# nv-legate/legate.sparse

Measured on AMD Instinct MI355X. Metric: cg_iters_per_sec, higher is better.
Workload: dtype fp64; 1 GPU; model=poisson2d-5pt-cg, nx=16384, n=268435456, nnz=1342111744, parallelism=dp1 1-D row partition + window gather

## Files before the change

### sparse/kernels/src/common.h

```cpp
#pragma once

#include <type_traits>

#include <hip/hip_runtime.h>

#include <ATen/ATen.h>
#include <ATen/Dispatch.h>
#include <ATen/hip/HIPContext.h>
#include <c10/util/complex.h>

#define SPARSE_CHECK_HIP(cmd)                                             \
  do {                                                                    \
    hipError_t e = (cmd);                                                 \
    TORCH_CHECK(e == hipSuccess, "HIP error: ", hipGetErrorString(e));    \
  } while (0)

constexpr int WAVE = 64;

__device__ __forceinline__ int64_t ub_i64(const int64_t* arr, int64_t n, int64_t key) {
  int64_t lo = 0, hi = n;
  while (lo < hi) {
    int64_t mid = (lo + hi) >> 1;
    if (arr[mid] <= key) lo = mid + 1; else hi = mid;
  }
  return lo;
}

__device__ __forceinline__ int64_t lb_i64(const int64_t* arr, int64_t n, int64_t key) {
  int64_t lo = 0, hi = n;
  while (lo < hi) {
    int64_t mid = (lo + hi) >> 1;
    if (arr[mid] < key) lo = mid + 1; else hi = mid;
  }
  return lo;
}

template <typename T>
__device__ __forceinline__ void atomic_add_any(T* addr, T v) {
  atomicAdd(addr, v);
}
template <typename T>
__device__ __forceinline__ void atomic_add_any(c10::complex<T>* addr, c10::complex<T> v) {
  T* p = reinterpret_cast<T*>(addr);
  atomicAdd(p, v.real());
  atomicAdd(p + 1, v.imag());
}

template <typename T>
struct ZeroOf { static __device__ __forceinline__ T value() { return T(0); } };
template <typename T>
struct ZeroOf<c10::complex<T>> {
  static __device__ __forceinline__ c10::complex<T> value() { return {T(0), T(0)}; }
};

#define DISPATCH_INDEX(ITYPE, NAME, ...)                       \
  [&] {                                                        \
    if ((ITYPE) == at::kInt) {                                 \
      using index_t = int32_t;                                 \
      return __VA_ARGS__();                                    \
    } else {                                                   \
      using index_t = int64_t;                                 \
      return __VA_ARGS__();                                    \
    }                                                          \
  }()

#define DISPATCH_VALUES(VTYPE, NAME, ...) \
  AT_DISPATCH_FLOATING_AND_COMPLEX_TYPES(VTYPE, NAME, __VA_ARGS__)

__device__ __forceinline__ int64_t xcd_swizzle(int64_t bid, int64_t nwg) {
  constexpr int64_t NXCD = 8;
  int64_t q = nwg / NXCD, rr = nwg % NXCD;
  int64_t xcd = bid % NXCD, idx = bid / NXCD;
  return (xcd < rr ? xcd * (q + 1) : rr * (q + 1) + (xcd - rr) * q) + idx;
}

inline hipStream_t cur_stream() {
  return c10::hip::getCurrentHIPStreamMasqueradingAsCUDA().stream();
}

template <typename T>
__device__ __forceinline__ T nt_load(const T* __restrict__ p) {
  if constexpr (std::is_arithmetic_v<T>) {
    return __builtin_nontemporal_load(p);
  } else {
    return *p;
  }
}
```

### sparse/kernels/src/elemwise.hip

```cpp
#include "common.h"

namespace {

template <typename index_t>
__global__ void add_nnz_kernel(const int64_t* __restrict__ aip,
                               const index_t* __restrict__ aix,
                               const int64_t* __restrict__ bip,
                               const index_t* __restrict__ bix,
                               int64_t* __restrict__ out, int64_t m) {
  int64_t r = (int64_t)blockIdx.x * blockDim.x + threadIdx.x;
  if (r >= m) return;
  int64_t pa = aip[r], ea = aip[r + 1];
  int64_t pb = bip[r], eb = bip[r + 1];
  int64_t c = 0;
  while (pa < ea && pb < eb) {
    index_t ca = aix[pa], cb = bix[pb];
    if (ca == cb) { ++pa; ++pb; }
    else if (ca < cb) ++pa;
    else ++pb;
    ++c;
  }
  out[r] = c + (ea - pa) + (eb - pb);
}

// ... 144 lines not shown
                         dim3(256), 0, cur_stream(), aip.data_ptr<int64_t>(),
                         aix.data_ptr<index_t>(), av.data_ptr<T>(),
                         bip.data_ptr<int64_t>(), bix.data_ptr<index_t>(),
                         bv.data_ptr<T>(), cip.data_ptr<int64_t>(),
                         cix.data_ptr<index_t>(), cv.data_ptr<T>(), m,
                         static_cast<T>(alpha), static_cast<T>(beta));
    });
  });
}

void mult_nnz_hip(at::Tensor aip, at::Tensor aix, at::Tensor bip, at::Tensor bix,
                  at::Tensor out) {
  int64_t m = out.numel();
  if (m == 0) return;
  DISPATCH_INDEX(aix.scalar_type(), "mult_nnz", [&] {
    hipLaunchKernelGGL((mult_nnz_kernel<index_t>), dim3((m + 255) / 256), dim3(256),
                       0, cur_stream(), aip.data_ptr<int64_t>(),
                       aix.data_ptr<index_t>(), bip.data_ptr<int64_t>(),
                       bix.data_ptr<index_t>(), out.data_ptr<int64_t>(), m);
  });
}

void mult_compute_hip(at::Tensor aip, at::Tensor aix, at::Tensor av,
                      at::Tensor bip, at::Tensor bix, at::Tensor bv,
                      at::Tensor cip, at::Tensor cix, at::Tensor cv) {
  int64_t m = aip.numel() - 1;
  if (m == 0) return;
  DISPATCH_VALUES(cv.scalar_type(), "mult_compute", [&] {
    using T = scalar_t;
    DISPATCH_INDEX(aix.scalar_type(), "mult_compute_idx", [&] {
      hipLaunchKernelGGL((mult_compute_kernel<T, index_t>), dim3((m + 255) / 256),
                         dim3(256), 0, cur_stream(), aip.data_ptr<int64_t>(),
                         aix.data_ptr<index_t>(), av.data_ptr<T>(),
                         bip.data_ptr<int64_t>(), bix.data_ptr<index_t>(),
                         bv.data_ptr<T>(), cip.data_ptr<int64_t>(),
                         cix.data_ptr<index_t>(), cv.data_ptr<T>(), m);
    });
  });
}

void mult_dense_hip(at::Tensor indptr, at::Tensor indices, at::Tensor vals,
                    at::Tensor D, at::Tensor out) {
  int64_t nnz = vals.numel();
  if (nnz == 0) return;
  int64_t m = indptr.numel() - 1;
  DISPATCH_VALUES(vals.scalar_type(), "mult_dense", [&] {
    using T = scalar_t;
    DISPATCH_INDEX(indices.scalar_type(), "mult_dense_idx", [&] {
      hipLaunchKernelGGL((mult_dense_kernel<T, index_t>), dim3((nnz + 255) / 256),
                         dim3(256), 0, cur_stream(), indptr.data_ptr<int64_t>(),
                         indices.data_ptr<index_t>(), vals.data_ptr<T>(),
                         D.data_ptr<T>(), out.data_ptr<T>(), m, D.size(1), nnz);
    });
  });
}

void axpby_hip(at::Tensor y, at::Tensor x, at::Tensor a, at::Tensor b,
               bool isalpha, bool negate) {
  int64_t n = y.numel();
  if (n == 0) return;
  const int64_t ept = std::max<int64_t>(1, 16 / y.element_size());
  int64_t blocks = (n / ept + 255) / 256 + 1;
  DISPATCH_VALUES(y.scalar_type(), "axpby", [&] {
    using T = scalar_t;
    auto launch = [&](auto kern) {
      hipLaunchKernelGGL(kern, dim3(blocks), dim3(256), 0, cur_stream(),
                         y.data_ptr<T>(), x.data_ptr<T>(), a.data_ptr<T>(),
                         b.data_ptr<T>(), n);
    };
    if (isalpha && !negate) launch(axpby_kernel<T, true, false>);
    else if (isalpha && negate) launch(axpby_kernel<T, true, true>);
    else if (!isalpha && !negate) launch(axpby_kernel<T, false, false>);
    else launch(axpby_kernel<T, false, true>);
  });
}

namespace {

template <typename T, bool ISALPHA, bool NEG>
__global__ __launch_bounds__(256) void axpby_norm2_kernel(
    T* __restrict__ y, const T* __restrict__ x, const T* __restrict__ a,
    const T* __restrict__ b, T* __restrict__ dot_partial, int64_t n) {
  constexpr int EPT = EptOf<T>::value;
  __shared__ T red[256];
  T s = (*a) / (*b);
  if (NEG) s = -s;
  T acc = T(0);
  const int64_t nv = n / EPT;
  const int64_t i = (int64_t)blockIdx.x * blockDim.x + threadIdx.x;
  if (i < nv) {
    auto* y2 = reinterpret_cast<VVec<T>*>(y);
    auto* x2 = reinterpret_cast<const VVec<T>*>(x);
    VVec<T> yv = y2[i];
    const VVec<T> xv = x2[i];
#pragma unroll
    for (int j = 0; j < EPT; ++j) {
      yv.v[j] = ISALPHA ? (yv.v[j] + s * xv.v[j]) : (xv.v[j] + s * yv.v[j]);
      acc += yv.v[j] * yv.v[j];
    }
    y2[i] = yv;
  }
  if (blockIdx.x == 0 && threadIdx.x == 0) {
    for (int64_t t = nv * EPT; t < n; ++t) {
      T v = ISALPHA ? (y[t] + s * x[t]) : (x[t] + s * y[t]);
      y[t] = v;
      acc += v * v;
    }
  }
  red[threadIdx.x] = acc;
  __syncthreads();
  for (int w = 128; w > 0; w >>= 1) {
    if (threadIdx.x < w) red[threadIdx.x] += red[threadIdx.x + w];
    __syncthreads();
  }
  if (threadIdx.x == 0) dot_partial[blockIdx.x] = red[0];
}

template <typename T>
__global__ __launch_bounds__(256) void cg_xr_norm2_kernel(
    T* __restrict__ x, const T* __restrict__ p, T* __restrict__ r,
    const T* __restrict__ q, const T* __restrict__ a, const T* __restrict__ b,
    T* __restrict__ dot_partial, int64_t n) {
  constexpr int EPT = EptOf<T>::value;
  __shared__ T red[256];
  const T s = (*a) / (*b);
  T acc = T(0);
  const int64_t nv = n / EPT;
  const int64_t i = (int64_t)blockIdx.x * blockDim.x + threadIdx.x;
  if (i < nv) {
    auto* x2 = reinterpret_cast<VVec<T>*>(x);
    auto* r2 = reinterpret_cast<VVec<T>*>(r);
    auto* p2 = reinterpret_cast<const VVec<T>*>(p);
    auto* q2 = reinterpret_cast<const VVec<T>*>(q);
    VVec<T> xv = x2[i];
    VVec<T> rv = r2[i];
    const VVec<T> pv = p2[i];
    const VVec<T> qv = q2[i];
#pragma unroll
    for (int j = 0; j < EPT; ++j) {
      xv.v[j] += s * pv.v[j];
      rv.v[j] -= s * qv.v[j];
      acc += rv.v[j] * rv.v[j];
    }
    x2[i] = xv;
    r2[i] = rv;
  }
  if (blockIdx.x == 0 && threadIdx.x == 0) {
    for (int64_t t = nv * EPT; t < n; ++t) {
      x[t] += s * p[t];
      const T rv = r[t] - s * q[t];
      r[t] = rv;
      acc += rv * rv;
    }
  }
  red[threadIdx.x] = acc;
  __syncthreads();
  for (int w = 128; w > 0; w >>= 1) {
    if ((int)threadIdx.x < w) red[threadIdx.x] += red[threadIdx.x + w];
    __syncthreads();
  }
  if (threadIdx.x == 0) dot_partial[blockIdx.x] = red[0];
}

}

void cg_xr_norm2_hip(at::Tensor x, at::Tensor p, at::Tensor r, at::Tensor q,
                     at::Tensor a, at::Tensor b, at::Tensor dot_out) {
  int64_t n = x.numel();
  if (n == 0) return;
  const int64_t ept = std::max<int64_t>(1, 16 / x.element_size());
  int64_t blocks = (n / ept + 255) / 256 + 1;
  TORCH_CHECK(dot_out.numel() >= blocks,
              "cg_xr_norm2: dot_out too small (", dot_out.numel(), " < ",
              blocks, ")");
  AT_DISPATCH_FLOATING_TYPES(x.scalar_type(), "cg_xr_norm2", [&] {
    using T = scalar_t;
    hipLaunchKernelGGL(cg_xr_norm2_kernel<T>, dim3(blocks), dim3(256), 0,
                       cur_stream(), x.data_ptr<T>(), p.data_ptr<T>(),
                       r.data_ptr<T>(), q.data_ptr<T>(), a.data_ptr<T>(),
                       b.data_ptr<T>(), dot_out.data_ptr<T>(), n);
  });
}

void axpby_norm2_hip(at::Tensor y, at::Tensor x, at::Tensor a, at::Tensor b,
                     bool isalpha, bool negate, at::Tensor dot_out) {
  int64_t n = y.numel();
  if (n == 0) return;
  const int64_t ept = std::max<int64_t>(1, 16 / y.element_size());
  int64_t blocks = (n / ept + 255) / 256 + 1;
  TORCH_CHECK(dot_out.numel() >= blocks,
              "axpby_norm2: dot_out too small (", dot_out.numel(), " < ",
              blocks, ")");
  AT_DISPATCH_FLOATING_TYPES(y.scalar_type(), "axpby_norm2", [&] {
    using T = scalar_t;
    auto launch = [&](auto kern) {
      hipLaunchKernelGGL(kern, dim3(blocks), dim3(256), 0, cur_stream(),
                         y.data_ptr<T>(), x.data_ptr<T>(), a.data_ptr<T>(),
                         b.data_ptr<T>(), dot_out.data_ptr<T>(), n);
    };
    if (isalpha && !negate) launch(axpby_norm2_kernel<T, true, false>);
    else if (isalpha && negate) launch(axpby_norm2_kernel<T, true, true>);
    else if (!isalpha && !negate) launch(axpby_norm2_kernel<T, false, false>);
    else launch(axpby_norm2_kernel<T, false, true>);
  });
}
```

### sparse/kernels/src/spmv.hip

```cpp
#include <type_traits>

#include "common.h"

namespace {

constexpr int BLK = 256;
constexpr int VT = 8;
constexpr int64_t NNZ_PER_BLOCK = (int64_t)BLK * VT;

template <typename U>
struct alignas(4 * sizeof(U) <= 16 ? 4 * sizeof(U) : 16) Quad {
  U v[4];
};

template <typename U>
struct alignas(2 * sizeof(U) <= 16 ? 2 * sizeof(U) : 16) Pair {
  U a, b;
};

template <typename T>
__device__ __forceinline__ void block_reduce_sum(T* red, int tid) {
  __syncthreads();
  for (int w = BLK / 2; w > 0; w >>= 1) {
    if (tid < w) red[tid] += red[tid + w];
// ... 341 lines not shown
          x0 = t.a;
          x1 = t.b;
        } else {
          x0 = own[c0];
          x1 = own[c0 + 1];
        }
      } else {
        x0 = own[min(max(c0, (int64_t)0), wsize - 1)];
        x1 = own[min(max(c0 + 1, (int64_t)0), wsize - 1)];
      }
    } else {
      x0 = at<false>(min(max(c0, (int64_t)0), wsize - 1));
      x1 = at<false>(min(max(c0 + 1, (int64_t)0), wsize - 1));
    }
  }
};

template <typename T, typename index_t, bool SINGLE>
__device__ __forceinline__ void ell_accumulate(
    const index_t* __restrict__ eidx, const T* __restrict__ evals, int W,
    int64_t mp, int64_t r0, int64_t col_lo, const XWindow<T>& win, T& a0,
    T& a1) {
  for (int k = 0; k < W; ++k) {
    const int64_t base = (int64_t)k * mp + r0;
    Pair<index_t> ii;
    ii.a = nt_load(&eidx[base]);
    ii.b = nt_load(&eidx[base + 1]);
    Pair<T> vv;
    vv.a = nt_load(&evals[base]);
    vv.b = nt_load(&evals[base + 1]);
    a0 += vv.a * win.template at<SINGLE>((int64_t)ii.a - col_lo);
    a1 += vv.b * win.template at<SINGLE>((int64_t)ii.b - col_lo);
  }
}

template <typename T>
struct DiaPlanes {
  static constexpr int kBatch = 1;
  const T* __restrict__ dvals;
  int64_t mp;

  struct Rows {
    const T* __restrict__ p;
    int64_t mp;
    __device__ __forceinline__ void at(int k, T& v0, T& v1) const {
      const int64_t base = (int64_t)k * mp;
      v0 = nt_load(&p[base]);
      v1 = nt_load(&p[base + 1]);
    }
  };
  __device__ __forceinline__ Rows rows(int64_t r0) const {
    return {dvals + r0, mp};
  }
};

template <int BYTES> struct UIntOf;
template <> struct UIntOf<2> { using type = uint16_t; };
template <> struct UIntOf<4> { using type = uint32_t; };
template <> struct UIntOf<8> { using type = uint64_t; };

template <typename T, typename M>
struct DiaConstPlanes {
  static constexpr int kBatch = 8;
  const T* __restrict__ cvals;
  const M* __restrict__ mask;

  struct Rows {
    const T* __restrict__ c;
    uint32_t m0, m1;
    __device__ __forceinline__ void at(int k, T& v0, T& v1) const {
      const T ck = c[k];
      const uint32_t bit = 1u << k;
      v0 = (m0 & bit) ? ck : T(0);
      v1 = (m1 & bit) ? ck : T(0);
    }
  };
  __device__ __forceinline__ Rows rows(int64_t r0) const {
    using M2 = typename UIntOf<2 * sizeof(M)>::type;
    const M2 w = nt_load(reinterpret_cast<const M2*>(&mask[r0]));
    return {cvals, (uint32_t)(M)w, (uint32_t)(w >> (8 * sizeof(M)))};
  }
};

template <typename T, typename Planes, typename XPair>
__device__ __forceinline__ void dia_accumulate(
    const Planes& planes, const int64_t* __restrict__ offs, int W, int64_t r0,
    int64_t cbase, XPair xpair, T& a0, T& a1) {
  const auto rows = planes.rows(r0);
  constexpr int U = Planes::kBatch;
  if constexpr (U == 1) {
    for (int k = 0; k < W; ++k) {
      T v0, v1;
      rows.at(k, v0, v1);
      T x0, x1;
      xpair(cbase + offs[k], x0, x1);
      a0 += v0 * x0;
      a1 += v1 * x1;
    }
  } else {
    for (int k = 0; k < W; k += U) {
      T x0[U], x1[U];
#pragma unroll
      for (int j = 0; j < U; ++j) {
        if (k + j < W) xpair(cbase + offs[k + j], x0[j], x1[j]);
      }
#pragma unroll
      for (int j = 0; j < U; ++j) {
        if (k + j < W) {
          T v0, v1;
          rows.at(k + j, v0, v1);
          a0 += v0 * x0[j];
          a1 += v1 * x1[j];
        }
      }
    }
  }
}

template <typename T>
__device__ __forceinline__ void store_pair_or_tail(T* __restrict__ dst,
                                                   int64_t r0, int64_t m,
                                                   int64_t rhi, T v0, T v1) {
  if (r0 + 1 < min(m, rhi)) {
    *reinterpret_cast<Pair<T>*>(&dst[r0]) = Pair<T>{v0, v1};
  } else if (r0 < m) {
    dst[r0] = v0;
  }
}

template <typename T>
__device__ __forceinline__ void jacobi_update(
    const T* __restrict__ xloc, const T* __restrict__ b,
    const T* __restrict__ dinv, T* __restrict__ xout, T omega, int64_t r0,
    int64_t m, int64_t rhi, T a0, T a1) {
  if (r0 + 1 < min(m, rhi)) {
    const Pair<T> xv = *reinterpret_cast<const Pair<T>*>(&xloc[r0]);
    const Pair<T> bv = *reinterpret_cast<const Pair<T>*>(&b[r0]);
    const Pair<T> dv = *reinterpret_cast<const Pair<T>*>(&dinv[r0]);
    *reinterpret_cast<Pair<T>*>(&xout[r0]) =
        Pair<T>{xv.a + omega * dv.a * (bv.a - a0),
                xv.b + omega * dv.b * (bv.b - a1)};
  } else if (r0 < m) {
    xout[r0] = xloc[r0] + omega * dinv[r0] * (b[r0] - a0);
  }
}

template <typename T>
__device__ __forceinline__ void block_dot_partial(T* red, T d,
                                                  T* __restrict__ dot_partial) {
  red[threadIdx.x] = d;
  block_reduce_sum(red, (int)threadIdx.x);
  if (threadIdx.x == 0) dot_partial[blockIdx.x] = red[0];
}

template <typename T, typename index_t, bool FUSE_DOT, bool SINGLE>
__global__ __launch_bounds__(BLK) void ell_spmv_kernel(
    const index_t* __restrict__ eidx, const T* __restrict__ evals,
    const XWindow<T> win, T* __restrict__ y, const T* __restrict__ pvec,
    T* __restrict__ dot_partial, int64_t m, int64_t mp, int W, int64_t col_lo,
    int64_t rbase, int64_t rhi) {
  __shared__ __align__(16) char red_raw[BLK * sizeof(T)];
  const int64_t r0 = rbase + 2 * ((int64_t)blockIdx.x * BLK + threadIdx.x);
  T a0 = ZeroOf<T>::value(), a1 = ZeroOf<T>::value();
  if (r0 < rhi) {
    ell_accumulate<T, index_t, SINGLE>(eidx, evals, W, mp, r0, col_lo, win,
                                       a0, a1);
    store_pair_or_tail(y, r0, m, rhi, a0, a1);
  }
  if (FUSE_DOT) {
    T d = ZeroOf<T>::value();
    if (r0 < min(m, rhi)) d += a0 * pvec[r0];
    if (r0 + 1 < min(m, rhi)) d += a1 * pvec[r0 + 1];
    block_dot_partial(reinterpret_cast<T*>(red_raw), d, dot_partial);
  }
}

template <typename T, typename index_t, bool SINGLE>
__global__ __launch_bounds__(BLK) void ell_jacobi_kernel(
    const index_t* __restrict__ eidx, const T* __restrict__ evals,
    const XWindow<T> win, const T* __restrict__ xloc,
    const T* __restrict__ b, const T* __restrict__ dinv,
    T* __restrict__ xout, int64_t m, int64_t mp, int W, int64_t col_lo,
    T omega) {
  const int64_t r0 = 2 * ((int64_t)blockIdx.x * BLK + threadIdx.x);
  if (r0 >= mp) return;
  T a0 = ZeroOf<T>::value(), a1 = ZeroOf<T>::value();
  ell_accumulate<T, index_t, SINGLE>(eidx, evals, W, mp, r0, col_lo, win, a0,
                                     a1);
  jacobi_update(xloc, b, dinv, xout, omega, r0, m, m, a0, a1);
}

template <typename T, typename Planes, bool FUSE_DOT, bool SINGLE,
          bool RESID = false>
__global__ __launch_bounds__(BLK) void dia_spmv_kernel(
    const Planes planes,
    const int64_t* __restrict__ offs,
    const XWindow<T> win, T* __restrict__ y, const T* __restrict__ pvec,
    T* __restrict__ dot_partial, int64_t m, int64_t mp, int W, int64_t col_lo,
    int64_t row0, int64_t rbase, int64_t rhi) {
  __shared__ __align__(16) char red_raw[BLK * sizeof(T)];
  const int64_t r0 = rbase + 2 * ((int64_t)blockIdx.x * BLK + threadIdx.x);
  T a0 = ZeroOf<T>::value(), a1 = ZeroOf<T>::value();
  if (r0 < rhi) {
    dia_accumulate(
        planes, offs, W, r0, row0 + r0 - col_lo,
        [&](int64_t c0, T& x0, T& x1) {
          win.template pair<SINGLE, Planes::kBatch != 1>(c0, x0, x1);
        },
        a0, a1);
    if (!RESID) {
      store_pair_or_tail(y, r0, m, rhi, a0, a1);
    } else if (r0 + 1 < min(m, rhi)) {
      const Pair<T> bv = *reinterpret_cast<const Pair<T>*>(&pvec[r0]);
      *reinterpret_cast<Pair<T>*>(&y[r0]) = Pair<T>{bv.a - a0, bv.b - a1};
    } else if (r0 < m) {
      y[r0] = pvec[r0] - a0;
    }
  }
  if (FUSE_DOT) {
    T d = ZeroOf<T>::value();
    if (r0 < min(m, rhi)) d += a0 * pvec[r0];
    if (r0 + 1 < min(m, rhi)) d += a1 * pvec[r0 + 1];
    block_dot_partial(reinterpret_cast<T*>(red_raw), d, dot_partial);
  }
}

template <typename T, typename Planes, bool SINGLE>
__global__ __launch_bounds__(BLK) void dia_jacobi_kernel(
    const Planes planes, const int64_t* __restrict__ offs,
    const XWindow<T> win, const T* __restrict__ xloc,
    const T* __restrict__ b, const T* __restrict__ dinv,
    T* __restrict__ xout, int64_t m, int64_t mp, int W, int64_t col_lo,
    int64_t row0, T omega, int64_t rbase, int64_t rhi) {
  const int64_t r0 = rbase + 2 * ((int64_t)blockIdx.x * BLK + threadIdx.x);
  if (r0 >= rhi) return;
  T a0 = ZeroOf<T>::value(), a1 = ZeroOf<T>::value();
  dia_accumulate(
      planes, offs, W, r0, row0 + r0 - col_lo,
      [&](int64_t c0, T& x0, T& x1) {
        win.template pair<SINGLE, Planes::kBatch != 1>(c0, x0, x1);
      },
      a0, a1);
  jacobi_update(xloc, b, dinv, xout, omega, r0, m, rhi, a0, a1);
}

template <typename T, typename Planes, bool SINGLE>
__global__ __launch_bounds__(BLK) void dia_spmv_bpdot_kernel(
    const Planes planes, const int64_t* __restrict__ offs,
    const XWindow<T> rwin, const XWindow<T> pwin, T* __restrict__ pnew,
    T* __restrict__ q, const T* __restrict__ beta_num,
    const T* __restrict__ beta_den, T* __restrict__ dot_partial, int64_t m,
    int64_t mp, int W, int64_t col_lo, int64_t row0) {
  __shared__ __align__(16) char red_raw[BLK * sizeof(T)];
  const T beta = (*beta_num) / (*beta_den);
  const int64_t r0 = 2 * ((int64_t)blockIdx.x * BLK + threadIdx.x);
  T a0 = ZeroOf<T>::value(), a1 = ZeroOf<T>::value();
  T p0 = ZeroOf<T>::value(), p1 = ZeroOf<T>::value();
  if (r0 < mp) {
    auto pnew_pair = [&](int64_t c0, T& x0, T& x1) {
      T r0v, r1v, p0v, p1v;
      rwin.template pair<SINGLE, Planes::kBatch != 1>(c0, r0v, r1v);
      pwin.template pair<SINGLE, Planes::kBatch != 1>(c0, p0v, p1v);
      x0 = r0v + beta * p0v;
      x1 = r1v + beta * p1v;
    };
    const int64_t cbase = row0 + r0 - col_lo;
    dia_accumulate(planes, offs, W, r0, cbase, pnew_pair, a0, a1);
    pnew_pair(cbase, p0, p1);
    store_pair_or_tail(pnew, r0, m, m, p0, p1);
    store_pair_or_tail(q, r0, m, m, a0, a1);
  }
  T d = ZeroOf<T>::value();
  if (r0 < m) d += a0 * p0;
  if (r0 + 1 < m) d += a1 * p1;
  block_dot_partial(reinterpret_cast<T*>(red_raw), d, dot_partial);
}

inline int64_t pair_blocks(int64_t span) {
  return (span + 2 * BLK - 1) / (2 * BLK);
}

template <typename F>
void dispatch_bool(bool v, F&& f) {
  if (v) f(std::true_type{}); else f(std::false_type{});
}

struct RowPairLaunch {
  int64_t mp, rbase, rhi, nlo, nown, wsize, nblocks;
  bool single;

  RowPairLaunch(int64_t mp_, const at::Tensor& hlo, const at::Tensor& own,
                const at::Tensor& hhi, int64_t wsize_, int64_t rbase_ = 0,
                int64_t rhi_ = -1)
      : mp(mp_), rbase(rbase_), rhi(rhi_ < 0 ? mp : rhi_),
        nlo(hlo.numel()), nown(own.numel()), wsize(wsize_),
        nblocks(rhi > rbase ? pair_blocks(rhi - rbase) : 0),
        single(nlo == 0 && hhi.numel() == 0) {}

  bool empty() const { return nblocks == 0; }

  template <typename T>
  XWindow<T> window(const at::Tensor& hlo, const at::Tensor& own,
                    const at::Tensor& hhi) const {
    const T* o = own.data_ptr<T>();
    return {hlo.numel() ? hlo.data_ptr<T>() : o, o,
            hhi.numel() ? hhi.data_ptr<T>() : o, nlo, nown, wsize};
  }

  template <typename... P, typename... A>
  void launch(void (*kern)(P...), A... args) const {
    hipLaunchKernelGGL(kern, dim3(nblocks), dim3(BLK), 0, cur_stream(),
                       static_cast<P>(args)...);
  }
};

using OptTensor = c10::optional<at::Tensor>;

inline int64_t dia_mp(const at::Tensor& planes, const OptTensor& mask,
                      int64_t W) {
  return mask ? mask->numel() : planes.numel() / W;
}

template <typename T, typename F>
void dispatch_dia_planes(const at::Tensor& planes, const OptTensor& mask,
                         int64_t W, F&& f) {
  if (!mask) {
    f(DiaPlanes<T>{planes.data_ptr<T>(), planes.numel() / W});
    return;
  }
  if constexpr (std::is_floating_point_v<T>) {
    TORCH_CHECK(planes.numel() == W && W <= 8 * (int64_t)mask->element_size() &&
                    mask->numel() % 2 == 0,
                "dia: W constants and an even number of mask words of at "
                "least W bits expected");
    const T* c = planes.data_ptr<T>();
    const void* mw = mask->data_ptr();
    switch (mask->scalar_type()) {
      case at::kByte:
        f(DiaConstPlanes<T, uint8_t>{c, static_cast<const uint8_t*>(mw)});
        return;
      case at::kUInt16:
        f(DiaConstPlanes<T, uint16_t>{c, static_cast<const uint16_t*>(mw)});
        return;
      case at::kUInt32:
        f(DiaConstPlanes<T, uint32_t>{c, static_cast<const uint32_t*>(mw)});
        return;
      default:
        break;
    }
  }
  TORCH_CHECK(false, "dia: constant planes need a real value type and a "
                     "uint8/uint16/uint32 row mask");
}

}

void build_ell_hip(at::Tensor indptr, at::Tensor indices, at::Tensor values,
                   at::Tensor eidx, at::Tensor evals, int64_t W,
                   int64_t pad_idx) {
  const int64_t m = indptr.numel() - 1;
  const int64_t mp = evals.numel() / W;
  DISPATCH_VALUES(values.scalar_type(), "build_ell", [&] {
    using T = scalar_t;
    DISPATCH_INDEX(indices.scalar_type(), "build_ell_idx", [&] {
      hipLaunchKernelGGL((build_ell_kernel<T, index_t>), dim3((mp + 255) / 256),
                         dim3(256), 0, cur_stream(), indptr.data_ptr<int64_t>(),
                         indices.data_ptr<index_t>(), values.data_ptr<T>(),
                         eidx.data_ptr<index_t>(), evals.data_ptr<T>(), m, mp,
                         (int)W, (index_t)pad_idx);
    });
  });
}

void build_dia_hip(at::Tensor indptr, at::Tensor indices, at::Tensor values,
                   at::Tensor offs, at::Tensor dvals, int64_t W,
                   int64_t row0) {
  const int64_t m = indptr.numel() - 1;
  const int64_t mp = dvals.numel() / W;
  if (m == 0) return;
  DISPATCH_VALUES(values.scalar_type(), "build_dia", [&] {
    using T = scalar_t;
    DISPATCH_INDEX(indices.scalar_type(), "build_dia_idx", [&] {
      hipLaunchKernelGGL((build_dia_kernel<T, index_t>),
                         dim3((m + 255) / 256), dim3(256), 0, cur_stream(),
                         indptr.data_ptr<int64_t>(),
                         indices.data_ptr<index_t>(), values.data_ptr<T>(),
                         offs.data_ptr<int64_t>(), dvals.data_ptr<T>(), m, mp,
                         (int)W, row0);
    });
  });
}

void dia_classify_hip(at::Tensor dvals, at::Tensor cvals, at::Tensor mask,
                      at::Tensor ok, int64_t W) {
  const int64_t mp = mask.numel();
  TORCH_CHECK(dvals.numel() == W * mp && cvals.numel() == W &&
                  cvals.scalar_type() == dvals.scalar_type() &&
                  ok.scalar_type() == at::kInt &&
                  W <= 8 * (int64_t)mask.element_size(),
              "dia_classify: inconsistent arguments");
  if (mp == 0) return;
  const dim3 g1((unsigned)std::min<int64_t>((mp + 255) / 256, 1024),
                (unsigned)W);
  auto run = [&](auto bits, auto word) {
    using B = decltype(bits);
    using M = decltype(word);
    const B* d = static_cast<const B*>(dvals.data_ptr());
    B* c = static_cast<B*>(cvals.data_ptr());
    hipLaunchKernelGGL((dia_plane_const_kernel<B>), g1, dim3(256), 0,
                       cur_stream(), d, c, mp);
    hipLaunchKernelGGL((dia_row_mask_kernel<B, M>), dim3((mp + 255) / 256),
                       dim3(256), 0, cur_stream(), d, c,
                       static_cast<M*>(mask.data_ptr()),
                       ok.data_ptr<int32_t>(), mp, (int)W);
  };
  auto by_word = [&](auto bits) {
    switch (mask.scalar_type()) {
      case at::kByte: run(bits, uint8_t{}); break;
      case at::kUInt16: run(bits, uint16_t{}); break;
      case at::kUInt32: run(bits, uint32_t{}); break;
      default: TORCH_CHECK(false, "dia_classify: mask must be uint8/16/32");
    }
  };
  switch (dvals.scalar_type()) {
    case at::kFloat: by_word(uint32_t{}); break;
    case at::kDouble: by_word(uint64_t{}); break;
    default: TORCH_CHECK(false, "dia_classify: fp32/fp64 planes only");
  }
}

static at::Tensor sum_or_zero(const at::Tensor& partial,
                              const at::Tensor& like) {
  return partial.defined() ? partial.sum() : at::zeros({}, like.options());
}

// ... 1 lines not shown
                                const at::Tensor& hlo, const at::Tensor& own,
                                const at::Tensor& hhi, at::Tensor& y,
                                const at::Tensor* pvec, int64_t W, int64_t m,
                                int64_t col_lo, int64_t rbase, int64_t rhi) {
  const RowPairLaunch L(evals.numel() / W, hlo, own, hhi, 0, rbase, rhi);
  at::Tensor partial;
  if (L.empty()) return partial;
  if (pvec) partial = at::empty({L.nblocks}, evals.options());
  DISPATCH_VALUES(evals.scalar_type(), "ell_spmv", [&] {
    using T = scalar_t;
    DISPATCH_INDEX(eidx.scalar_type(), "ell_spmv_idx", [&] {
      dispatch_bool(pvec != nullptr, [&](auto fuse) {
        dispatch_bool(L.single, [&](auto single) {
          L.launch(ell_spmv_kernel<T, index_t, decltype(fuse)::value,
                                   decltype(single)::value>,
                   eidx.data_ptr<index_t>(), evals.data_ptr<T>(),
                   L.window<T>(hlo, own, hhi), y.data_ptr<T>(),
                   pvec ? pvec->data_ptr<T>() : nullptr,
                   pvec ? partial.data_ptr<T>() : nullptr, m, L.mp, W, col_lo,
                   L.rbase, L.rhi);
        });
      });
    });
  });
  return partial;
}

void ell_spmv_plain_hip(at::Tensor eidx, at::Tensor evals, at::Tensor hlo,
                        at::Tensor own, at::Tensor hhi, at::Tensor y,
                        int64_t W, int64_t m, int64_t col_lo,
                        int64_t rbase, int64_t rhi) {
  ell_spmv_impl(eidx, evals, hlo, own, hhi, y, nullptr, W, m, col_lo, rbase,
                rhi);
}

at::Tensor ell_spmv_dot_hip(at::Tensor eidx, at::Tensor evals, at::Tensor hlo,
                            at::Tensor own, at::Tensor hhi, at::Tensor y,
                            at::Tensor pvec, int64_t W, int64_t m,
                            int64_t col_lo, int64_t rbase, int64_t rhi) {
  return sum_or_zero(ell_spmv_impl(eidx, evals, hlo, own, hhi, y, &pvec, W, m,
                                   col_lo, rbase, rhi),
                     evals);
}

void ell_jacobi_hip(at::Tensor eidx, at::Tensor evals, at::Tensor hlo,
                    at::Tensor own, at::Tensor hhi, at::Tensor xloc,
                    at::Tensor b, at::Tensor dinv, at::Tensor xout,
                    int64_t W, int64_t m, int64_t col_lo, double omega) {
  const RowPairLaunch L(evals.numel() / W, hlo, own, hhi, 0);
  if (L.empty()) return;
  DISPATCH_VALUES(evals.scalar_type(), "ell_jacobi", [&] {
    using T = scalar_t;
    DISPATCH_INDEX(eidx.scalar_type(), "ell_jacobi_idx", [&] {
      dispatch_bool(L.single, [&](auto single) {
        L.launch(ell_jacobi_kernel<T, index_t, decltype(single)::value>,
                 eidx.data_ptr<index_t>(), evals.data_ptr<T>(),
                 L.window<T>(hlo, own, hhi), xloc.data_ptr<T>(),
                 b.data_ptr<T>(), dinv.data_ptr<T>(), xout.data_ptr<T>(), m,
                 L.mp, W, col_lo, omega);
      });
    });
  });
}

template <bool RESID>
static at::Tensor dia_spmv_impl(const at::Tensor& planes, const OptTensor& mask,
                                const at::Tensor& offs, const at::Tensor& hlo,
                                const at::Tensor& own, const at::Tensor& hhi,
                                at::Tensor& y, const at::Tensor* pvec,
                                int64_t W, int64_t m, int64_t col_lo,
                                int64_t row0, int64_t wsize, int64_t rbase,
                                int64_t rhi) {
  const RowPairLaunch L(dia_mp(planes, mask, W), hlo, own, hhi, wsize, rbase,
                        rhi);
  const bool fuse_dot = pvec && !RESID;
  at::Tensor partial;
  if (L.empty()) return partial;
  if (fuse_dot) partial = at::empty({L.nblocks}, planes.options());
  DISPATCH_VALUES(planes.scalar_type(), "dia_spmv", [&] {
    using T = scalar_t;
    dispatch_dia_planes<T>(planes, mask, W, [&](auto pl) {
      dispatch_bool(fuse_dot, [&](auto fuse) {
        dispatch_bool(L.single, [&](auto single) {
          if constexpr (!(RESID && decltype(fuse)::value)) {
            L.launch(dia_spmv_kernel<T, decltype(pl), decltype(fuse)::value,
                                     decltype(single)::value, RESID>,
                     pl, offs.data_ptr<int64_t>(), L.window<T>(hlo, own, hhi),
                     y.data_ptr<T>(), pvec ? pvec->data_ptr<T>() : nullptr,
                     fuse_dot ? partial.data_ptr<T>() : nullptr, m, L.mp, W,
                     col_lo, row0, L.rbase, L.rhi);
          }
        });
      });
    });
  });
  return partial;
}

void dia_spmv_plain_hip(at::Tensor planes, OptTensor mask, at::Tensor offs,
                        at::Tensor hlo, at::Tensor own, at::Tensor hhi,
                        at::Tensor y, int64_t W, int64_t m, int64_t col_lo,
                        int64_t row0, int64_t wsize, int64_t rbase,
                        int64_t rhi) {
  dia_spmv_impl<false>(planes, mask, offs, hlo, own, hhi, y, nullptr, W, m,
                       col_lo, row0, wsize, rbase, rhi);
}

at::Tensor dia_spmv_dot_hip(at::Tensor planes, OptTensor mask, at::Tensor offs,
                            at::Tensor hlo, at::Tensor own, at::Tensor hhi,
                            at::Tensor y, at::Tensor pvec, int64_t W,
                            int64_t m, int64_t col_lo, int64_t row0,
                            int64_t wsize, int64_t rbase, int64_t rhi) {
  return sum_or_zero(dia_spmv_impl<false>(planes, mask, offs, hlo, own, hhi, y,
                                          &pvec, W, m, col_lo, row0, wsize,
                                          rbase, rhi),
                     planes);
}

void dia_residual_hip(at::Tensor planes, OptTensor mask, at::Tensor offs,
                      at::Tensor hlo, at::Tensor own, at::Tensor hhi,
                      at::Tensor b, at::Tensor y, int64_t W, int64_t m,
                      int64_t col_lo, int64_t row0, int64_t wsize,
                      int64_t rbase, int64_t rhi) {
  dia_spmv_impl<true>(planes, mask, offs, hlo, own, hhi, y, &b, W, m, col_lo,
                      row0, wsize, rbase, rhi);
}

void dia_jacobi_hip(at::Tensor planes, OptTensor mask, at::Tensor offs,
                    at::Tensor hlo, at::Tensor own, at::Tensor hhi,
                    at::Tensor xloc, at::Tensor b, at::Tensor dinv,
                    at::Tensor xout, int64_t W, int64_t m, int64_t col_lo,
                    int64_t row0, int64_t wsize, double omega, int64_t rbase,
                    int64_t rhi) {
  const RowPairLaunch L(dia_mp(planes, mask, W), hlo, own, hhi, wsize, rbase,
                        rhi);
  if (L.empty()) return;
  DISPATCH_VALUES(planes.scalar_type(), "dia_jacobi", [&] {
    using T = scalar_t;
    dispatch_dia_planes<T>(planes, mask, W, [&](auto pl) {
      dispatch_bool(L.single, [&](auto single) {
        L.launch(dia_jacobi_kernel<T, decltype(pl), decltype(single)::value>,
                 pl, offs.data_ptr<int64_t>(), L.window<T>(hlo, own, hhi),
                 xloc.data_ptr<T>(), b.data_ptr<T>(), dinv.data_ptr<T>(),
                 xout.data_ptr<T>(), m, L.mp, W, col_lo, row0, omega, L.rbase,
                 L.rhi);
      });
    });
  });
}

at::Tensor dia_spmv_bpdot_hip(at::Tensor planes, OptTensor mask,
                              at::Tensor offs, at::Tensor r_hlo,
                              at::Tensor r_own, at::Tensor r_hhi,
                              at::Tensor p_hlo, at::Tensor p_own,
                              at::Tensor p_hhi, at::Tensor pnew, at::Tensor q,
                              at::Tensor beta_num, at::Tensor beta_den,
                              int64_t W, int64_t m, int64_t col_lo,
                              int64_t row0, int64_t wsize) {
  TORCH_CHECK(pnew.data_ptr() != p_own.data_ptr(),
              "dia_spmv_bpdot: pnew must not alias p_own (double-buffer)");
  const RowPairLaunch L(dia_mp(planes, mask, W), r_hlo, r_own, r_hhi, wsize);
  at::Tensor partial;
  if (L.empty()) return sum_or_zero(partial, planes);
  partial = at::empty({L.nblocks}, planes.options());
  DISPATCH_VALUES(planes.scalar_type(), "dia_spmv_bpdot", [&] {
    using T = scalar_t;
    dispatch_dia_planes<T>(planes, mask, W, [&](auto pl) {
      dispatch_bool(L.single, [&](auto single) {
        L.launch(dia_spmv_bpdot_kernel<T, decltype(pl), decltype(single)::value>,
                 pl, offs.data_ptr<int64_t>(),
                 L.window<T>(r_hlo, r_own, r_hhi),
                 L.window<T>(p_hlo, p_own, p_hhi), pnew.data_ptr<T>(),
                 q.data_ptr<T>(), beta_num.data_ptr<T>(),
                 beta_den.data_ptr<T>(), partial.data_ptr<T>(), m, L.mp, W,
                 col_lo, row0);
      });
    });
  });
  return partial.sum();
}
```

Baseline: 210.0 iters/s.

## Add specialized constant-plane DIA kernels with compile-time width and multi-pair rows

Adds dedicated SpMV, Jacobi and fused bpdot kernels for DIA matrices stored as constant coefficients plus a row bitmask. The diagonal count is a template parameter (1-8 for uint8 masks), each thread handles several row pairs, and an interior fast path loads x windows as aligned pairs without per-element bounds checks. Block reductions switch from a shared-memory tree to wave shuffles, and explicit FMAs are used throughout. The goal is to cut index, bounds and reduction overhead in the bandwidth-bound 5-point stencil SpMV, at the cost of more template instantiations and higher register pressure.

```diff
diff --git a/sparse/kernels/src/common.h b/sparse/kernels/src/common.h
--- a/sparse/kernels/src/common.h
+++ b/sparse/kernels/src/common.h
@@ -74,6 +74,37 @@
   return (xcd < rr ? xcd * (q + 1) : rr * (q + 1) + (xcd - rr) * q) + idx;
 }
 
+template <typename T>
+__device__ __forceinline__ T wave_reduce_sum(T v) {
+#pragma unroll
+  for (int off = WAVE / 2; off > 0; off >>= 1) v += __shfl_down(v, off, WAVE);
+  return v;
+}
+template <typename T>
+__device__ __forceinline__ c10::complex<T> wave_reduce_sum(c10::complex<T> v) {
+  return {wave_reduce_sum(v.real()), wave_reduce_sum(v.imag())};
+}
+
+template <int N = 1, typename T>
+__device__ __forceinline__ T block_sums_256(const T (&v)[N]) {
+  constexpr int NW = 256 / WAVE;
+  __shared__ __align__(16) char raw[N * NW * sizeof(T)];
+  T* ws = reinterpret_cast<T*>(raw);
+  const int lane = threadIdx.x % WAVE, wid = threadIdx.x / WAVE;
+#pragma unroll
+  for (int n = 0; n < N; ++n) {
+    const T s = wave_reduce_sum(v[n]);
+    if (lane == 0) ws[n * NW + wid] = s;
+  }
+  __syncthreads();
+  T s = ZeroOf<T>::value();
+  if (threadIdx.x < N) {
+    const T* w = ws + threadIdx.x * NW;
+    s = ((w[0] + w[1]) + w[2]) + w[3];
+  }
+  return s;
+}
+
 inline hipStream_t cur_stream() {
   return c10::hip::getCurrentHIPStreamMasqueradingAsCUDA().stream();
 }
diff --git a/sparse/kernels/src/elemwise.hip b/sparse/kernels/src/elemwise.hip
--- a/sparse/kernels/src/elemwise.hip
+++ b/sparse/kernels/src/elemwise.hip
@@ -250,7 +250,6 @@
     T* __restrict__ y, const T* __restrict__ x, const T* __restrict__ a,
     const T* __restrict__ b, T* __restrict__ dot_partial, int64_t n) {
   constexpr int EPT = EptOf<T>::value;
-  __shared__ T red[256];
   T s = (*a) / (*b);
   if (NEG) s = -s;
   T acc = T(0);
@@ -275,13 +274,9 @@
       acc += v * v;
     }
   }
-  red[threadIdx.x] = acc;
-  __syncthreads();
-  for (int w = 128; w > 0; w >>= 1) {
-    if (threadIdx.x < w) red[threadIdx.x] += red[threadIdx.x + w];
-    __syncthreads();
-  }
-  if (threadIdx.x == 0) dot_partial[blockIdx.x] = red[0];
+  const T part[1] = {acc};
+  const T sum = block_sums_256(part);
+  if (threadIdx.x == 0) dot_partial[blockIdx.x] = sum;
 }
 
 template <typename T>
@@ -290,7 +285,6 @@
     const T* __restrict__ q, const T* __restrict__ a, const T* __restrict__ b,
     T* __restrict__ dot_partial, int64_t n) {
   constexpr int EPT = EptOf<T>::value;
-  __shared__ T red[256];
   const T s = (*a) / (*b);
   T acc = T(0);
   const int64_t nv = n / EPT;
@@ -321,13 +315,9 @@
       acc += rv * rv;
     }
   }
-  red[threadIdx.x] = acc;
-  __syncthreads();
-  for (int w = 128; w > 0; w >>= 1) {
-    if ((int)threadIdx.x < w) red[threadIdx.x] += red[threadIdx.x + w];
-    __syncthreads();
-  }
-  if (threadIdx.x == 0) dot_partial[blockIdx.x] = red[0];
+  const T part[1] = {acc};
+  const T sum = block_sums_256(part);
+  if (threadIdx.x == 0) dot_partial[blockIdx.x] = sum;
 }
 
 }
diff --git a/sparse/kernels/src/spmv.hip b/sparse/kernels/src/spmv.hip
--- a/sparse/kernels/src/spmv.hip
+++ b/sparse/kernels/src/spmv.hip
@@ -447,6 +447,17 @@
   }
 };
 
+template <typename T>
+__device__ __forceinline__ T fmadd(T v, T x, T a) {
+  if constexpr (std::is_same_v<T, float>) {
+    return __builtin_fmaf(v, x, a);
+  } else if constexpr (std::is_same_v<T, double>) {
+    return __builtin_fma(v, x, a);
+  } else {
+    return a + v * x;
+  }
+}
+
 template <typename T, typename Planes, typename XPair>
 __device__ __forceinline__ void dia_accumulate(
     const Planes& planes, const int64_t* __restrict__ offs, int W, int64_t r0,
@@ -459,8 +470,8 @@
       rows.at(k, v0, v1);
       T x0, x1;
       xpair(cbase + offs[k], x0, x1);
-      a0 += v0 * x0;
-      a1 += v1 * x1;
+      a0 = fmadd(v0, x0, a0);
+      a1 = fmadd(v1, x1, a1);
     }
   } else {
     for (int k = 0; k < W; k += U) {
@@ -474,8 +485,8 @@
         if (k + j < W) {
           T v0, v1;
           rows.at(k + j, v0, v1);
-          a0 += v0 * x0[j];
-          a1 += v1 * x1[j];
+          a0 = fmadd(v0, x0[j], a0);
+          a1 = fmadd(v1, x1[j], a1);
         }
       }
     }
@@ -503,19 +514,19 @@
     const Pair<T> bv = *reinterpret_cast<const Pair<T>*>(&b[r0]);
     const Pair<T> dv = *reinterpret_cast<const Pair<T>*>(&dinv[r0]);
     *reinterpret_cast<Pair<T>*>(&xout[r0]) =
-        Pair<T>{xv.a + omega * dv.a * (bv.a - a0),
-                xv.b + omega * dv.b * (bv.b - a1)};
+        Pair<T>{fmadd(omega * dv.a, bv.a - a0, xv.a),
+                fmadd(omega * dv.b, bv.b - a1, xv.b)};
   } else if (r0 < m) {
-    xout[r0] = xloc[r0] + omega * dinv[r0] * (b[r0] - a0);
+    xout[r0] = fmadd(omega * dinv[r0], b[r0] - a0, xloc[r0]);
   }
 }
 
 template <typename T>
-__device__ __forceinline__ void block_dot_partial(T* red, T d,
+__device__ __forceinline__ void block_dot_partial(T d,
                                                   T* __restrict__ dot_partial) {
-  red[threadIdx.x] = d;
-  block_reduce_sum(red, (int)threadIdx.x);
-  if (threadIdx.x == 0) dot_partial[blockIdx.x] = red[0];
+  const T part[1] = {d};
+  const T sum = block_sums_256(part);
+  if (threadIdx.x == 0) dot_partial[blockIdx.x] = sum;
 }
 
 template <typename T, typename index_t, bool FUSE_DOT, bool SINGLE>
@@ -524,7 +535,6 @@
     const XWindow<T> win, T* __restrict__ y, const T* __restrict__ pvec,
     T* __restrict__ dot_partial, int64_t m, int64_t mp, int W, int64_t col_lo,
     int64_t rbase, int64_t rhi) {
-  __shared__ __align__(16) char red_raw[BLK * sizeof(T)];
   const int64_t r0 = rbase + 2 * ((int64_t)blockIdx.x * BLK + threadIdx.x);
   T a0 = ZeroOf<T>::value(), a1 = ZeroOf<T>::value();
   if (r0 < rhi) {
@@ -536,7 +546,7 @@
     T d = ZeroOf<T>::value();
     if (r0 < min(m, rhi)) d += a0 * pvec[r0];
     if (r0 + 1 < min(m, rhi)) d += a1 * pvec[r0 + 1];
-    block_dot_partial(reinterpret_cast<T*>(red_raw), d, dot_partial);
+    block_dot_partial(d, dot_partial);
   }
 }
 
@@ -563,7 +573,6 @@
     const XWindow<T> win, T* __restrict__ y, const T* __restrict__ pvec,
     T* __restrict__ dot_partial, int64_t m, int64_t mp, int W, int64_t col_lo,
     int64_t row0, int64_t rbase, int64_t rhi) {
-  __shared__ __align__(16) char red_raw[BLK * sizeof(T)];
   const int64_t r0 = rbase + 2 * ((int64_t)blockIdx.x * BLK + threadIdx.x);
   T a0 = ZeroOf<T>::value(), a1 = ZeroOf<T>::value();
   if (r0 < rhi) {
@@ -584,9 +593,9 @@
   }
   if (FUSE_DOT) {
     T d = ZeroOf<T>::value();
-    if (r0 < min(m, rhi)) d += a0 * pvec[r0];
-    if (r0 + 1 < min(m, rhi)) d += a1 * pvec[r0 + 1];
-    block_dot_partial(reinterpret_cast<T*>(red_raw), d, dot_partial);
+    if (r0 < min(m, rhi)) d = fmadd(a0, pvec[r0], d);
+    if (r0 + 1 < min(m, rhi)) d = fmadd(a1, pvec[r0 + 1], d);
+    block_dot_partial(d, dot_partial);
   }
 }
 
@@ -616,7 +625,6 @@
     T* __restrict__ q, const T* __restrict__ beta_num,
     const T* __restrict__ beta_den, T* __restrict__ dot_partial, int64_t m,
     int64_t mp, int W, int64_t col_lo, int64_t row0) {
-  __shared__ __align__(16) char red_raw[BLK * sizeof(T)];
   const T beta = (*beta_num) / (*beta_den);
   const int64_t r0 = 2 * ((int64_t)blockIdx.x * BLK + threadIdx.x);
   T a0 = ZeroOf<T>::value(), a1 = ZeroOf<T>::value();
@@ -626,8 +634,8 @@
       T r0v, r1v, p0v, p1v;
       rwin.template pair<SINGLE, Planes::kBatch != 1>(c0, r0v, r1v);
       pwin.template pair<SINGLE, Planes::kBatch != 1>(c0, p0v, p1v);
-      x0 = r0v + beta * p0v;
-      x1 = r1v + beta * p1v;
+      x0 = fmadd(beta, p0v, r0v);
+      x1 = fmadd(beta, p1v, r1v);
     };
     const int64_t cbase = row0 + r0 - col_lo;
     dia_accumulate(planes, offs, W, r0, cbase, pnew_pair, a0, a1);
@@ -636,9 +644,263 @@
     store_pair_or_tail(q, r0, m, m, a0, a1);
   }
   T d = ZeroOf<T>::value();
-  if (r0 < m) d += a0 * p0;
-  if (r0 + 1 < m) d += a1 * p1;
-  block_dot_partial(reinterpret_cast<T*>(red_raw), d, dot_partial);
+  if (r0 < m) d = fmadd(a0, p0, d);
+  if (r0 + 1 < m) d = fmadd(a1, p1, d);
+  block_dot_partial(d, dot_partial);
+}
+
+constexpr int kDiaPairs = 2;
+constexpr int kDiaBpdotPairs = 1;
+
+template <int WC, int R, bool SINGLE, int NWIN, typename T, typename M,
+          typename Comb, typename Pre, typename Post>
+__device__ __forceinline__ void dia_const_rows(
+    const DiaConstPlanes<T, M>& planes, const int64_t* __restrict__ offs,
+    int Wrt, const XWindow<T>& win0, const XWindow<T>& win1, Comb comb,
+    int64_t m, int64_t row0, int64_t col_lo, int64_t rbase, int64_t rhi,
+    Pre pre, Post post) {
+  constexpr int KB = WC ? WC : 8;
+  constexpr int64_t S = 2 * (int64_t)BLK * R;
+  const int W = WC ? WC : Wrt;
+  const int64_t lim = min(m, rhi);
+  const int64_t rb = rbase + (int64_t)blockIdx.x * S;
+  const int64_t t2 = 2 * (int64_t)threadIdx.x;
+  const int64_t cb = row0 + rb - col_lo - win0.nlo;
+  const int64_t own_end = min(win0.nown, win0.wsize - win0.nlo);
+  int64_t o[KB];
+  T c[KB];
+#pragma unroll
+  for (int i = 0; i < KB; ++i) {
+    if (i < W) {
+      o[i] = offs[i];
+      c[i] = planes.cvals[i];
+    }
+  }
+  const bool interior = rb + S <= lim && cb + o[0] >= 0 &&
+                        cb + (S - 1) + (WC ? o[KB - 1] : offs[W - 1]) < own_end;
+  if (interior) {
+    using M2 = typename UIntOf<2 * sizeof(M)>::type;
+    M2 mw[R];
+#pragma unroll
+    for (int j = 0; j < R; ++j) {
+      mw[j] = nt_load(
+          reinterpret_cast<const M2*>(planes.mask + rb + t2 + j * 2 * BLK));
+    }
+    T a[R][2];
+#pragma unroll
+    for (int j = 0; j < R; ++j) a[j][0] = a[j][1] = ZeroOf<T>::value();
+    for (int k0 = 0; k0 < W; k0 += KB) {
+      if (k0 > 0) {
+#pragma unroll
+        for (int i = 0; i < KB; ++i) {
+          if (k0 + i < W) {
+            o[i] = offs[k0 + i];
+            c[i] = planes.cvals[k0 + i];
+          }
+        }
+      }
+      T xv[NWIN][R][KB][2];
+#pragma unroll
+      for (int i = 0; i < KB; ++i) {
+        if (k0 + i < W) {
+#pragma unroll
+          for (int w = 0; w < NWIN; ++w) {
+            const T* ub = (w == 0 ? win0 : win1).own + (cb + o[i]);
+            const bool aligned =
+                (reinterpret_cast<uintptr_t>(ub) % sizeof(Pair<T>)) == 0;
+#pragma unroll
+            for (int j = 0; j < R; ++j) {
+              const T* p = ub + t2 + j * 2 * BLK;
+              if (aligned) {
+                const Pair<T> t = *reinterpret_cast<const Pair<T>*>(p);
+                xv[w][j][i][0] = t.a;
+                xv[w][j][i][1] = t.b;
+              } else {
+                xv[w][j][i][0] = p[0];
+                xv[w][j][i][1] = p[1];
+              }
+            }
+          }
+        }
+      }
+      if (k0 == 0) {
+#pragma unroll
+        for (int j = 0; j < R; ++j) pre(j, rb + t2 + j * 2 * BLK, true);
+        __builtin_amdgcn_sched_barrier(0);
+      }
+#pragma unroll
+      for (int j = 0; j < R; ++j) {
+        const uint32_t m0 = (uint32_t)(M)mw[j];
+        const uint32_t m1 = (uint32_t)(mw[j] >> (8 * sizeof(M)));
+#pragma unroll
+        for (int i = 0; i < KB; ++i) {
+          if (k0 + i < W) {
+            T v0[NWIN], v1[NWIN];
+#pragma unroll
+            for (int w = 0; w < NWIN; ++w) {
+              v0[w] = xv[w][j][i][0];
+              v1[w] = xv[w][j][i][1];
+            }
+            const uint32_t bit = 1u << (k0 + i);
+            a[j][0] = fmadd((m0 & bit) ? c[i] : T(0), comb(v0), a[j][0]);
+            a[j][1] = fmadd((m1 & bit) ? c[i] : T(0), comb(v1), a[j][1]);
+          }
+        }
+      }
+    }
+#pragma unroll
+    for (int j = 0; j < R; ++j) {
+      post(j, rb + t2 + j * 2 * BLK, a[j][0], a[j][1], true);
+    }
+  } else {
+#pragma unroll
+    for (int j = 0; j < R; ++j) {
+      const int64_t r0 = rb + t2 + j * 2 * BLK;
+      if (r0 < rhi) {
+        T a0 = ZeroOf<T>::value(), a1 = ZeroOf<T>::value();
+        pre(j, r0, r0 + 1 < lim);
+        dia_accumulate(
+            planes, offs, W, r0, row0 + r0 - col_lo,
+            [&](int64_t c0, T& x0, T& x1) {
+              T v0[NWIN], v1[NWIN];
+#pragma unroll
+              for (int w = 0; w < NWIN; ++w) {
+                (w == 0 ? win0 : win1)
+                    .template pair<SINGLE, true>(c0, v0[w], v1[w]);
+              }
+              x0 = comb(v0);
+              x1 = comb(v1);
+            },
+            a0, a1);
+        post(j, r0, a0, a1, r0 + 1 < lim);
+      }
+    }
+  }
+}
+
+template <typename T, typename M, int WC, bool FUSE_DOT, bool SINGLE,
+          bool RESID>
+__global__ __launch_bounds__(BLK) void dia_const_spmv_kernel(
+    const DiaConstPlanes<T, M> planes, const int64_t* __restrict__ offs,
+    const XWindow<T> win, T* __restrict__ y, const T* __restrict__ pvec,
+    T* __restrict__ dot_partial, int64_t m, int W, int64_t col_lo,
+    int64_t row0, int64_t rbase, int64_t rhi) {
+  constexpr int R = kDiaPairs;
+  const int64_t lim = min(m, rhi);
+  Pair<T> pv[R];
+  T d[R];
+#pragma unroll
+  for (int j = 0; j < R; ++j) {
+    pv[j] = Pair<T>{T(0), T(0)};
+    d[j] = T(0);
+  }
+  dia_const_rows<WC, R, SINGLE, 1>(
+      planes, offs, W, win, win, [](const T(&v)[1]) { return v[0]; }, m,
+      row0, col_lo, rbase, rhi,
+      [&](int j, int64_t r0, bool full) {
+        if (FUSE_DOT || RESID) {
+          if (full) {
+            pv[j] = *reinterpret_cast<const Pair<T>*>(&pvec[r0]);
+          } else if (r0 < lim) {
+            pv[j].a = pvec[r0];
+          }
+        }
+      },
+      [&](int j, int64_t r0, T a0, T a1, bool full) {
+        if (RESID) {
+          a0 = pv[j].a - a0;
+          a1 = pv[j].b - a1;
+        }
+        if (full) {
+          *reinterpret_cast<Pair<T>*>(&y[r0]) = Pair<T>{a0, a1};
+        } else {
+          store_pair_or_tail(y, r0, m, rhi, a0, a1);
+        }
+        if (FUSE_DOT) {
+          T dd = T(0);
+          if (full || r0 < lim) dd = fmadd(a0, pv[j].a, dd);
+          if (full) dd = fmadd(a1, pv[j].b, dd);
+          d[j] = dd;
+        }
+      });
+  if (FUSE_DOT) {
+    const T sum = block_sums_256<R>(d);
+    const int64_t slot = (int64_t)blockIdx.x * R + threadIdx.x;
+    if (threadIdx.x < R && slot * (2 * BLK) < rhi - rbase) {
+      dot_partial[slot] = sum;
+    }
+  }
+}
+
+template <typename T, typename M, int WC, bool SINGLE>
+__global__ __launch_bounds__(BLK) void dia_const_jacobi_kernel(
+    const DiaConstPlanes<T, M> planes, const int64_t* __restrict__ offs,
+    const XWindow<T> win, const T* __restrict__ xloc,
+    const T* __restrict__ b, const T* __restrict__ dinv,
+    T* __restrict__ xout, int64_t m, int W, int64_t col_lo, int64_t row0,
+    T omega, int64_t rbase, int64_t rhi) {
+  constexpr int R = kDiaPairs;
+  Pair<T> xv[R], bv[R], dv[R];
+  dia_const_rows<WC, R, SINGLE, 1>(
+      planes, offs, W, win, win, [](const T(&v)[1]) { return v[0]; }, m,
+      row0, col_lo, rbase, rhi,
+      [&](int j, int64_t r0, bool full) {
+        if (full) {
+          xv[j] = *reinterpret_cast<const Pair<T>*>(&xloc[r0]);
+          bv[j] = *reinterpret_cast<const Pair<T>*>(&b[r0]);
+          dv[j] = *reinterpret_cast<const Pair<T>*>(&dinv[r0]);
+        }
+      },
+      [&](int j, int64_t r0, T a0, T a1, bool full) {
+        if (full) {
+          *reinterpret_cast<Pair<T>*>(&xout[r0]) =
+              Pair<T>{fmadd(omega * dv[j].a, bv[j].a - a0, xv[j].a),
+                      fmadd(omega * dv[j].b, bv[j].b - a1, xv[j].b)};
+        } else {
+          jacobi_update(xloc, b, dinv, xout, omega, r0, m, rhi, a0, a1);
+        }
+      });
+}
+
+template <typename T, typename M, int WC, bool SINGLE>
+__global__ __launch_bounds__(BLK) void dia_const_bpdot_kernel(
+    const DiaConstPlanes<T, M> planes, const int64_t* __restrict__ offs,
+    const XWindow<T> rwin, const XWindow<T> pwin, T* __restrict__ pnew,
+    T* __restrict__ q, const T* __restrict__ beta_num,
+    const T* __restrict__ beta_den, T* __restrict__ dot_partial, int64_t m,
+    int64_t mp, int W, int64_t col_lo, int64_t row0) {
+  constexpr int R = kDiaBpdotPairs;
+  const T beta = (*beta_num) / (*beta_den);
+  auto comb = [&](const T(&v)[2]) { return fmadd(beta, v[1], v[0]); };
+  T rr[R][2], pp[R][2];
+  T d[R];
+#pragma unroll
+  for (int j = 0; j < R; ++j) d[j] = T(0);
+  dia_const_rows<WC, R, SINGLE, 2>(
+      planes, offs, W, rwin, pwin, comb, m, row0, col_lo, 0, mp,
+      [&](int j, int64_t r0, bool) {
+        const int64_t c0 = row0 + r0 - col_lo;
+        rwin.template pair<SINGLE, true>(c0, rr[j][0], rr[j][1]);
+        pwin.template pair<SINGLE, true>(c0, pp[j][0], pp[j][1]);
+      },
+      [&](int j, int64_t r0, T a0, T a1, bool full) {
+        const T v0[2] = {rr[j][0], pp[j][0]}, v1[2] = {rr[j][1], pp[j][1]};
+        const T p0 = comb(v0), p1 = comb(v1);
+        if (full) {
+          *reinterpret_cast<Pair<T>*>(&pnew[r0]) = Pair<T>{p0, p1};
+          *reinterpret_cast<Pair<T>*>(&q[r0]) = Pair<T>{a0, a1};
+        } else {
+          store_pair_or_tail(pnew, r0, m, m, p0, p1);
+          store_pair_or_tail(q, r0, m, m, a0, a1);
+        }
+        T dd = T(0);
+        if (full || r0 < m) dd = fmadd(a0, p0, dd);
+        if (full) dd = fmadd(a1, p1, dd);
+        d[j] = dd;
+      });
+  const T sum = block_sums_256<R>(d);
+  const int64_t slot = (int64_t)blockIdx.x * R + threadIdx.x;
+  if (threadIdx.x < R && slot * (2 * BLK) < mp) dot_partial[slot] = sum;
 }
 
 inline int64_t pair_blocks(int64_t span) {
@@ -676,6 +938,12 @@
   void launch(void (*kern)(P...), A... args) const {
     hipLaunchKernelGGL(kern, dim3(nblocks), dim3(BLK), 0, cur_stream(),
                        static_cast<P>(args)...);
+  }
+
+  template <int R, typename... P, typename... A>
+  void launch_pairs(void (*kern)(P...), A... args) const {
+    hipLaunchKernelGGL(kern, dim3((nblocks + R - 1) / R), dim3(BLK), 0,
+                       cur_stream(), static_cast<P>(args)...);
   }
 };
 
@@ -716,6 +984,29 @@
   }
   TORCH_CHECK(false, "dia: constant planes need a real value type and a "
                      "uint8/uint16/uint32 row mask");
+}
+
+template <typename P>
+struct DiaConstOf : std::false_type {};
+template <typename T, typename M>
+struct DiaConstOf<DiaConstPlanes<T, M>> : std::true_type {
+  using mask_t = M;
+};
+
+template <typename M, typename F>
+void dispatch_dia_wc(int64_t W, F&& f) {
+  TORCH_CHECK(W >= 1, "dia: at least one diagonal expected");
+  if constexpr (std::is_same_v<M, uint8_t>) {
+    switch (W) {
+#define SPARSE_DIA_WC(N) \
+  case N: f(std::integral_constant<int, N>{}); return;
+      SPARSE_DIA_WC(1) SPARSE_DIA_WC(2) SPARSE_DIA_WC(3) SPARSE_DIA_WC(4)
+      SPARSE_DIA_WC(5) SPARSE_DIA_WC(6) SPARSE_DIA_WC(7) SPARSE_DIA_WC(8)
+#undef SPARSE_DIA_WC
+      default: break;
+    }
+  }
+  f(std::integral_constant<int, 0>{});
 }
 
 }
@@ -883,13 +1174,27 @@
     dispatch_dia_planes<T>(planes, mask, W, [&](auto pl) {
       dispatch_bool(fuse_dot, [&](auto fuse) {
         dispatch_bool(L.single, [&](auto single) {
-          if constexpr (!(RESID && decltype(fuse)::value)) {
-            L.launch(dia_spmv_kernel<T, decltype(pl), decltype(fuse)::value,
+          using PL = decltype(pl);
+          const T* pp = pvec ? pvec->data_ptr<T>() : nullptr;
+          T* dp = fuse_dot ? partial.data_ptr<T>() : nullptr;
+          if constexpr (RESID && decltype(fuse)::value) {
+          } else if constexpr (DiaConstOf<PL>::value) {
+            using M = typename DiaConstOf<PL>::mask_t;
+            dispatch_dia_wc<M>(W, [&](auto wc) {
+              L.launch_pairs<kDiaPairs>(
+                  dia_const_spmv_kernel<T, M, decltype(wc)::value,
+                                        decltype(fuse)::value,
+                                        decltype(single)::value, RESID>,
+                  pl, offs.data_ptr<int64_t>(), L.window<T>(hlo, own, hhi),
+                  y.data_ptr<T>(), pp, dp, m, W, col_lo, row0, L.rbase,
+                  L.rhi);
+            });
+          } else {
+            L.launch(dia_spmv_kernel<T, PL, decltype(fuse)::value,
                                      decltype(single)::value, RESID>,
                      pl, offs.data_ptr<int64_t>(), L.window<T>(hlo, own, hhi),
-                     y.data_ptr<T>(), pvec ? pvec->data_ptr<T>() : nullptr,
-                     fuse_dot ? partial.data_ptr<T>() : nullptr, m, L.mp, W,
-                     col_lo, row0, L.rbase, L.rhi);
+                     y.data_ptr<T>(), pp, dp, m, L.mp, W, col_lo, row0,
+                     L.rbase, L.rhi);
           }
         });
       });
@@ -940,11 +1245,25 @@
     using T = scalar_t;
     dispatch_dia_planes<T>(planes, mask, W, [&](auto pl) {
       dispatch_bool(L.single, [&](auto single) {
-        L.launch(dia_jacobi_kernel<T, decltype(pl), decltype(single)::value>,
-                 pl, offs.data_ptr<int64_t>(), L.window<T>(hlo, own, hhi),
-                 xloc.data_ptr<T>(), b.data_ptr<T>(), dinv.data_ptr<T>(),
-                 xout.data_ptr<T>(), m, L.mp, W, col_lo, row0, omega, L.rbase,
-                 L.rhi);
+        using PL = decltype(pl);
+        if constexpr (DiaConstOf<PL>::value) {
+          using M = typename DiaConstOf<PL>::mask_t;
+          dispatch_dia_wc<M>(W, [&](auto wc) {
+            L.launch_pairs<kDiaPairs>(
+                dia_const_jacobi_kernel<T, M, decltype(wc)::value,
+                                        decltype(single)::value>,
+                pl, offs.data_ptr<int64_t>(), L.window<T>(hlo, own, hhi),
+                xloc.data_ptr<T>(), b.data_ptr<T>(), dinv.data_ptr<T>(),
+                xout.data_ptr<T>(), m, W, col_lo, row0, omega, L.rbase,
+                L.rhi);
+          });
+        } else {
+          L.launch(dia_jacobi_kernel<T, PL, decltype(single)::value>, pl,
+                   offs.data_ptr<int64_t>(), L.window<T>(hlo, own, hhi),
+                   xloc.data_ptr<T>(), b.data_ptr<T>(), dinv.data_ptr<T>(),
+                   xout.data_ptr<T>(), m, L.mp, W, col_lo, row0, omega,
+                   L.rbase, L.rhi);
+        }
       });
     });
   });
@@ -968,13 +1287,26 @@
     using T = scalar_t;
     dispatch_dia_planes<T>(planes, mask, W, [&](auto pl) {
       dispatch_bool(L.single, [&](auto single) {
-        L.launch(dia_spmv_bpdot_kernel<T, decltype(pl), decltype(single)::value>,
-                 pl, offs.data_ptr<int64_t>(),
+        using PL = decltype(pl);
+        auto go = [&](auto launch, auto kern) {
+          launch(kern, pl, offs.data_ptr<int64_t>(),
                  L.window<T>(r_hlo, r_own, r_hhi),
                  L.window<T>(p_hlo, p_own, p_hhi), pnew.data_ptr<T>(),
                  q.data_ptr<T>(), beta_num.data_ptr<T>(),
                  beta_den.data_ptr<T>(), partial.data_ptr<T>(), m, L.mp, W,
                  col_lo, row0);
+        };
+        if constexpr (DiaConstOf<PL>::value) {
+          using M = typename DiaConstOf<PL>::mask_t;
+          dispatch_dia_wc<M>(W, [&](auto wc) {
+            go([&](auto... a) { L.launch_pairs<kDiaBpdotPairs>(a...); },
+               dia_const_bpdot_kernel<T, M, decltype(wc)::value,
+                                      decltype(single)::value>);
+          });
+        } else {
+          go([&](auto... a) { L.launch(a...); },
+             dia_spmv_bpdot_kernel<T, PL, decltype(single)::value>);
+        }
       });
     });
   });
```

New measurement: 225.1 iters/s, median of 6. 7.2% higher.
